# lalitkrajendran/photon

Hardware: AMD Instinct MI355X
Metric: Mrays/sec, 1e7-ray 256^3 BOS render (higher is better)
Workload: dtype f32

## Files before the change

### photon_amd/csrc/device_volume_coop.hpp

```cpp
#pragma once
#include "../../include/photon_philox.h"
#include "device_volume.hpp"

namespace photon {

enum PathSlot : int {
    PS_C_COHERENT,
    PS_C_HIT_CELL,
    PS_C_CELL_IN_TILE,
    PS_C_FETCH_UP,
    PS_C_FETCH_DOWN,
    PS_C_TILE_CLAMPED,
    PS_C_INCOHERENT,
    PS_C_INCOHERENT_LANES,
    PS_C_BRICK_PASS,
    PS_C_BRICK_FETCH,
    PS_C_BRICK_REUSED,
    PS_C_BRICK_CLAMPED,
    PS_C_BRICK_LANES,
    PS_C_GATHER_LANES,
    PS_C_SPIN_OUTSIDE,
    PS_C_SPIN_LOW,
    PS_C_SPIN_CAP,
    PS_L_COHERENT,
    PS_L_HIT_A,
    PS_L_HIT_B,
    PS_L_TILE_B_LANES,
    PS_L_FETCH,
    PS_L_FETCH_TWO,
    PS_L_FETCH_TO_B,
    PS_L_FETCH_DOWN,
    PS_L_BASE_AHEAD,
    PS_L_BASE_BEHIND,
    PS_L_TILE_CLAMPED,
    PS_L_NO_FREE_TILE,
    PS_L_OUT_OF_REACH,
    PS_L_MARK_INCOHERENT,
    PS_L_TILES_SKIPPED,
    PS_L_RETRY,
    PS_L_COHERENT_AGAIN,
    PS_L_INCOHERENT,
    PS_L_INCOHERENT_LANES,
    PS_L_BRICK_PASS,
    PS_L_BRICK_FETCH,
    PS_L_BRICK_REUSED,
    PS_L_BRICK_CLAMPED,
    PS_L_BRICK_LANES,
    PS_L_GATHER_LANES,
    PS_L_SPIN_OUTSIDE,
    PS_L_SPIN_CAP,
    PS_L_LOW,
    PS_L_REPAIR_LANES,
    PS_L_KEEP_PREV_LANES,
    PS_COUNT
};
constexpr int kPathSlots = PS_COUNT;
#ifndef PHOTON_PATH_STATS
#define PHOTON_PATH_STATS 0
#endif
#if PHOTON_PATH_STATS
__device__ unsigned long long g_path_stats[kPathSlots];
__device__ __forceinline__ void path_stat(PathSlot k, unsigned long long n = 1) {
    if ((int)(threadIdx.x & 63) == __ffsll((long long)ballot(true)) - 1) atomicAdd(&g_path_stats[k], n);
}
__device__ __forceinline__ void path_stat_if(PathSlot k, bool c) { if (c) path_stat(k); }
__device__ __forceinline__ void path_lanes(PathSlot k, unsigned long long mask) { if (mask != 0) path_stat(k, (unsigned long long)__popcll(mask)); }
#else
#define path_stat(...) ((void)0)
#define path_stat_if(...) ((void)0)
#define path_lanes(...) ((void)0)
#endif

#ifndef PHOTON_BRICK_PASSES
#define PHOTON_BRICK_PASSES 6
#endif
#ifndef PHOTON_LINEAR_TILE_LAYERS
#define PHOTON_LINEAR_TILE_LAYERS 16
#endif
#ifndef PHOTON_LINEAR_TILES
#define PHOTON_LINEAR_TILES 2
#endif
#ifndef PHOTON_TILE_RETRY_MASK
#define PHOTON_TILE_RETRY_MASK 15
#endif
#ifndef PHOTON_BRICK_PITCH
#define PHOTON_BRICK_PITCH 12
// ... 192 lines not shown
    }
#if PHOTON_PRIO_TAPS_DPP != PHOTON_PRIO_TAPS_LDS
    __builtin_amdgcn_s_setprio(PHOTON_PRIO_TAPS_LDS);
#endif
    f4 t[4] = {f4{t0.x, t0.y, t0.z, t0.w}, f4{t1.x, t1.y, t1.z, t1.w}, f4{t2.x, t2.y, t2.z, t2.w}, f4{t3.x, t3.y, t3.z, t3.w}};
    float w0 = wxy[0][0];
#pragma unroll
    for (int r = R; r < 16; r++) {
        const int b = r & 3, c = r >> 2;
#pragma unroll
        for (int a = 0; a < 4; a++) {
            const f4 ta = t[a];
            const float w = (a == 0 && b == 0) ? w0 : wxy[b][a];
            if (a == 0 && b == 0) s = f4{w * ta.x, w * ta.y, w * ta.z, w * ta.w};
            else s = f4{fmaf(w, ta.x, s.x), fmaf(w, ta.y, s.y), fmaf(w, ta.z, s.z), fmaf(w, ta.w, s.w)};
            asm volatile("" : "+v"(s.x), "+v"(s.y), "+v"(s.z), "+v"(s.w) : : "memory");
            if (r < 15) t[a] = ldtexel(blk + ((r + 1) >> 2) * 16 + ((r + 1) & 3) * 4 + a);
            asm volatile("" : "+v"(w0) : : "memory");
        }
        if (b == 3) {
            if (c == 0) acc = f4{wz[0] * s.x, wz[0] * s.y, wz[0] * s.z, wz[0] * s.w};
            else acc = f4{fmaf(wz[c], s.x, acc.x), fmaf(wz[c], s.y, acc.y), fmaf(wz[c], s.z, acc.z), fmaf(wz[c], s.w, acc.w)};
            asm volatile("" : "+v"(acc.x), "+v"(acc.y), "+v"(acc.z), "+v"(acc.w) : : "memory");
        }
    }
#if PHOTON_PRIO_TAPS_LDS != PHOTON_PRIO_BASE
    __builtin_amdgcn_s_setprio(PHOTON_PRIO_BASE);
#endif
    return acc;
}

__device__ __forceinline__ bool lane_of(unsigned long long mask) { return __builtin_amdgcn_inverse_ballot_w64(mask); }

struct Parked { int ti, tj, tk; int bi, bj, bk; f4 reg; int ci, cj, k0, coff; int ui, uj, uk; f4 more[3]; };
__device__ __forceinline__ Parked parked_none() {
    return Parked{0x7fffffff, 0x7fffffff, 0x7fffffff, 0x7fffffff, 0x7fffffff, 0x7fffffff, f4{0, 0, 0, 0}, 0x7fffffff, 0x7fffffff, 0, 0, 0x7fffffff, 0x7fffffff, 0x7fffffff, {f4{0, 0, 0, 0}, f4{0, 0, 0, 0}, f4{0, 0, 0, 0}}};
}

struct Lead { int i, j, k; };
__device__ __forceinline__ Lead lead_of(unsigned long long todo, float fi, float fj, float fk) {
    const int leader = __ffsll((long long)todo) - 1;
    return Lead{__builtin_amdgcn_readlane(__float_as_int(fi), leader), __builtin_amdgcn_readlane(__float_as_int(fj), leader),
                __builtin_amdgcn_readlane(__float_as_int(fk), leader)};
}
__device__ __forceinline__ unsigned long long same_block(const Lead &c, float fi, float fj, float fk) {
    return ballot(__float_as_int(fi) == c.i) & ballot(__float_as_int(fj) == c.j) & ballot(__float_as_int(fk) == c.k);
}

__device__ __forceinline__ f4 tex3d_cubic_coop(const VolumeDev &v, const f4 *__restrict__ tex, f4 *blk, unsigned long long need,
                                               float x, float y, float z, Parked &parked) {
    f4 *const brick = blk + tile_texels<2>();
    const float xg = x - 0.5f, yg = y - 0.5f, zg = z - 0.5f;
    const float fi = floorf(xg), fj = floorf(yg), fk = floorf(zg);
    float wx[4], wy[4], wz[4];
    bspline_weights(xg - fi, wx[0], wx[1], wx[2], wx[3]);
    bspline_weights(yg - fj, wy[0], wy[1], wy[2], wy[3]);
    bspline_weights(zg - fk, wz[0], wz[1], wz[2], wz[3]);
    const int lane = threadIdx.x & 63;
    if (need == 0) return f4{0, 0, 0, 0};
    {
        constexpr int TL = kCubicTileLayers;
        bool hit = false;
        if (parked.ti != 0x7fffffff) {
            asm volatile("");
            hit = ((ballot(__float_as_int(fi) == parked.ti) & ballot(__float_as_int(fj) == parked.tj) & ballot(__float_as_int(fk) == parked.tk)) & need) == need;
            path_stat_if(PS_C_HIT_CELL, hit);
        }
        if (!hit) {
            const Lead c = lead_of(need, fi, fj, fk);
            if ((same_block(c, fi, fj, fk) & need) == need) {
                const int ck = (int)__int_as_float(c.k);
                int dz = ck - parked.k0;
                if (c.i != parked.ci || c.j != parked.cj || (unsigned)dz > (unsigned)(TL - 4)) {
                    const int ci = (int)__int_as_float(c.i), cj = (int)__int_as_float(c.j);
                    const bool down = c.i == parked.ci && c.j == parked.cj && dz < 0;
                    const int k0 = down ? ck - (TL - 4) : ck;
                    path_stat(down ? PS_C_FETCH_DOWN : PS_C_FETCH_UP);
                    path_stat_if(PS_C_TILE_CLAMPED, ci < 1 || ci + 2 > v.nx - 1 || cj < 1 || cj + 2 > v.ny - 1 || k0 < 1 || k0 + TL - 2 > v.nz - 1);
                    __builtin_amdgcn_wave_barrier();
                    int l = lane;
                    asm volatile("" : "+v"(l));
                    const int tx = clampi(ci - 1 + (l & 3), 0, v.nx - 1), ty = clampi(cj - 1 + ((l >> 2) & 3), 0, v.ny - 1);
#pragma unroll
                    for (int j = 0; j < (TL + 3) / 4; j++) {
                        if (TL % 4 == 0 || j < TL / 4 || l < 16 * (TL % 4)) {
                            const int tz = clampi(k0 - 1 + (l >> 4) + 4 * j, 0, v.nz - 1);
                            const f4 t = ldtexel(tex + (unsigned)((tz * v.ny + ty) * v.nx + tx));
                            *reinterpret_cast<float4 *>(blk + l + 64 * j) = make_float4(t.x, t.y, t.z, t.w);
                        }
                    }
                    __builtin_amdgcn_wave_barrier();
                    parked.ci = c.i; parked.cj = c.j; parked.k0 = k0;
                    dz = ck - k0;
                } else {
                    path_stat(PS_C_CELL_IN_TILE);
                }
                parked.coff = dz * 16;
                parked.reg = ldtexel(blk + parked.coff + (lane & 15));
#pragma unroll
                for (int z = 1; z < kDppSlabs; z++) parked.more[z - 1] = ldtexel(blk + parked.coff + 16 * z + (lane & 15));
                parked.ti = c.i; parked.tj = c.j; parked.tk = c.k;
                hit = true;
            }
        }
        if (hit) {
            path_stat(PS_C_COHERENT);
            const f4 *cell = blk + parked.coff;
            const f4 acc = cubic_taps_hybrid(cell, parked.reg, parked.more, wx, wy, wz);
            __builtin_amdgcn_wave_barrier();
            return acc;
        }
        parked.ti = 0x7fffffff;
    }
    const int bi = (int)fi, bj = (int)fj, bk = (int)fk;
    f4 acc = f4{0, 0, 0, 0};
    bool done = !lane_of(need);
    unsigned long long todo = need;
    path_stat(PS_C_INCOHERENT);
    path_lanes(PS_C_INCOHERENT_LANES, need);
#pragma unroll 1
    for (int pass = 0; pass < PHOTON_BRICK_PASSES && todo != 0; pass++) {
        const int leader = __ffsll((long long)todo) - 1;
        const int ci = __builtin_amdgcn_readlane(bi, leader), cj = __builtin_amdgcn_readlane(bj, leader),
                  ck = __builtin_amdgcn_readlane(bk, leader);
        const int di = bi - ci + 2, dj = bj - cj + 2;
        const bool in_brick = !done && bk == ck && (unsigned)di <= 4u && (unsigned)dj <= 4u;
        path_stat(PS_C_BRICK_PASS);
        path_lanes(PS_C_BRICK_LANES, ballot(in_brick));
        path_stat(ci != parked.bi || cj != parked.bj || ck != parked.bk ? PS_C_BRICK_FETCH : PS_C_BRICK_REUSED);
        if (ci != parked.bi || cj != parked.bj || ck != parked.bk) {
            path_stat_if(PS_C_BRICK_CLAMPED, ci < 3 || ci + 4 > v.nx - 1 || cj < 3 || cj + 4 > v.ny - 1 || ck < 1 || ck + 2 > v.nz - 1);
            __builtin_amdgcn_wave_barrier();
            int l = lane;
            asm volatile("" : "+v"(l));
            const int slot = (l & 7) + ((l >> 3) & 7) * kBrickPitch;
#pragma unroll
            for (int j = 0; j < 4; j++) {
                const int t = l + 64 * j;
                const int tx = clampi(ci - 3 + (t & 7), 0, v.nx - 1), ty = clampi(cj - 3 + ((t >> 3) & 7), 0, v.ny - 1),
                          tz = clampi(ck - 1 + (t >> 6), 0, v.nz - 1);
// ... 27 lines not shown
    const float fi = floorf(xb), fj = floorf(yb), fk = floorf(zb);
    const float a = quant_weight(xb - fi, weight_scale, weight_inv), b = quant_weight(yb - fj, weight_scale, weight_inv),
                c = quant_weight(zb - fk, weight_scale, weight_inv);
    const int i = (int)fi, j = (int)fj, k = (int)fk;
    const int i0 = clampi(i, 0, nx - 1), i1 = clampi(i + 1, 0, nx - 1);
    const int j0 = clampi(j, 0, ny - 1), j1 = clampi(j + 1, 0, ny - 1);
    const int k0 = clampi(k, 0, nz - 1), k1 = clampi(k + 1, 0, nz - 1);
    auto row = [&](int kk, int jj) {
        const f4 *r = tex + (unsigned)((kk * ny + jj) * nx);
        f4 v = lerp4(ldtexel(r + i0), ldtexel(r + i1), a);
        asm volatile("" : "+v"(v.x), "+v"(v.y), "+v"(v.z), "+v"(v.w));
        return v;
    };
    const f4 c00 = row(k0, j0), c10 = row(k0, j1);
    f4 c0 = lerp4(c00, c10, b);
    asm volatile("" : "+v"(c0.x), "+v"(c0.y), "+v"(c0.z), "+v"(c0.w));
    const f4 c01 = row(k1, j0), c11 = row(k1, j1);
    const f4 c1 = lerp4(c01, c11, b);
    return lerp4(c0, c1, c);
}

__device__ __forceinline__ float uniformf(float x) {
    float s;
    asm("s_nop 0\n\tv_readfirstlane_b32 %0, %1\n\ts_nop 4" : "=s"(s) : "v"(x));
    return s;
}

__device__ __forceinline__ float pair_swap(float v) {
    return __int_as_float(__builtin_amdgcn_update_dpp(0, __float_as_int(v), 0xB1 , 0xF, 0xF, false));
}

template <bool QUANT, bool PIN = false>
__device__ __forceinline__ f4 tex3d_linear_coop(const VolumeDev &v, const f4 *__restrict__ tex, f4 *blk, unsigned long long need,
                                                float x, float y, float z, Parked &parked, unsigned tick = 0) {
    f4 *const brick = blk + tile_texels<1>();
    const float xb = x - 0.5f, yb = y - 0.5f, zb = z - 0.5f;
    const float fi = floorf(xb), fj = floorf(yb), fk = floorf(zb);
    float a = xb - fi, b = yb - fj, c = zb - fk;
    if (QUANT) {
        a = floorf(fmaf(a, v.weight_scale, 0.5f)) * v.weight_inv;

        b = floorf(fmaf(b, v.weight_scale, 0.5f)) * v.weight_inv;
        c = floorf(fmaf(c, v.weight_scale, 0.5f)) * v.weight_inv;
    }
    const int lane = threadIdx.x & 63;
    if (need == 0) return f4{0, 0, 0, 0};
    {
        constexpr int TL = PHOTON_LINEAR_TILE_LAYERS;
        constexpr int NT = PHOTON_LINEAR_TILES;
        static_assert(TL == 4 || TL == 8 || TL == 16, "PHOTON_LINEAR_TILE_LAYERS");
        static_assert(NT == 1 || NT == 2, "PHOTON_LINEAR_TILES");
        constexpr unsigned kDzMax = (unsigned)(TL - 2);
        constexpr int kIncoherent = 0x7ffffffe;
        const int fib = __float_as_int(fi), fjb = __float_as_int(fj);
        unsigned dzq = 0;
        unsigned long long ok_a = 0, ok_b = 0;
        bool hit = false;
        if (parked.ti != 0x7fffffff) {
            asm volatile("");
            dzq = (unsigned)(int)(fk - __int_as_float(parked.tk));
            ok_a = ballot(fib == parked.ti) & ballot(fjb == parked.tj) & ballot(dzq <= kDzMax);
            hit = (ok_a & need) == need;
            path_stat_if(PS_L_HIT_A, hit);
            if (NT == 2 && !hit && parked.ui < kIncoherent) {
                const unsigned dzu = (unsigned)(int)(fk - __int_as_float(parked.uk));
                ok_b = ballot(fib == parked.ui) & ballot(fjb == parked.uj) & ballot(dzu <= kDzMax);
                if (((ok_a | ok_b) & need) == need) {
                    hit = true;
                    path_stat(PS_L_HIT_B);
                    dzq = lane_of(ok_a) ? dzq : dzu + TL;
                }
            }
        }
        path_stat_if(PS_L_TILES_SKIPPED, !hit && parked.ui == kIncoherent && (tick & (unsigned)PHOTON_TILE_RETRY_MASK) != 0);
        path_stat_if(PS_L_RETRY, !hit && parked.ui == kIncoherent && (tick & (unsigned)PHOTON_TILE_RETRY_MASK) == 0);
        if (!hit && (parked.ui != kIncoherent || (tick & (unsigned)PHOTON_TILE_RETRY_MASK) == 0)) {
            const unsigned long long rest = need & ~(ok_a | ok_b);
            const Lead l1 = lead_of(rest, fi, fj, fk);
            const unsigned long long col1 = rest & ballot(fib == l1.i) & ballot(fjb == l1.j), rest2 = rest & ~col1;
            Lead l2 = l1;
            unsigned long long col2 = 0;
            int n_new = 1;
            if (rest2 != 0) {
                l2 = lead_of(rest2, fi, fj, fk);
                col2 = rest2 & ballot(fib == l2.i) & ballot(fjb == l2.j);
                n_new = (rest2 & ~col2) != 0 ? 3 : 2;
            }
            const bool free_a = (ok_a & need) == 0, free_b = NT == 2 && (ok_b & need) == 0;
            path_stat_if(PS_L_NO_FREE_TILE, n_new > (free_a ? 1 : 0) + (free_b ? 1 : 0));
            if (n_new <= (free_a ? 1 : 0) + (free_b ? 1 : 0)) {
                path_stat_if(PS_L_FETCH_TWO, n_new == 2);
#pragma unroll 1
                for (int j = 0; j < n_new; j++) {
                    path_stat(PS_L_FETCH);
                    const bool to_a = j == 0 && free_a;
                    const Lead ld = j == 0 ? l1 : l2;
                    const unsigned long long lanes = j == 0 ? col1 : col2;
                    const int oi = to_a ? parked.ti : parked.ui, oj = to_a ? parked.tj : parked.uj, ok = to_a ? parked.tk : parked.uk;
                    const float klf = __int_as_float(ld.k);
                    const bool behind = (lanes & ballot(fk < klf)) != 0, ahead = (lanes & ballot(fk > klf)) != 0;
                    const bool down = ld.i == oi && ld.j == oj && klf < __int_as_float(ok);
                    const int ci = (int)__int_as_float(ld.i), cj = (int)__int_as_float(ld.j);
                    const int base = (int)klf - (down ? (ahead ? TL - 3 : TL - 2) : (behind ? 1 : 0));
                    f4 *const tile = blk + (to_a ? 0 : 4 * TL);
                    path_stat_if(PS_L_FETCH_TO_B, !to_a);
                    path_stat_if(PS_L_FETCH_DOWN, down);
                    path_stat_if(PS_L_BASE_AHEAD, down && ahead);
                    path_stat_if(PS_L_BASE_BEHIND, !down && behind);
                    path_stat_if(PS_L_TILE_CLAMPED, ci < 0 || ci + 1 > v.nx - 1 || cj < 0 || cj + 1 > v.ny - 1 || base < 0 || base + TL - 1 > v.nz - 1);
                    __builtin_amdgcn_wave_barrier();
                    if (lane < 4 * TL) {
                        int l = lane;
                        if (PIN) asm volatile("" : "+v"(l));
                        const int tx = clampi(ci + (l & 1), 0, v.nx - 1), ty = clampi(cj + ((l >> 1) & 1), 0, v.ny - 1),
                                  tz = clampi(base + (l >> 2), 0, v.nz - 1);
                        const f4 t = ldtexel(tex + (unsigned)((tz * v.ny + ty) * v.nx + tx));
                        const f4 o = f4{pair_swap(t.x), pair_swap(t.y), pair_swap(t.z), pair_swap(t.w)};
                        const bool hi = (l & 1) != 0;
                        *reinterpret_cast<float4 *>(tile + l) = make_float4(hi ? t.x - o.x : t.x, hi ? t.y - o.y : t.y,
                                                                            hi ? t.z - o.z : t.z, hi ? t.w - o.w : t.w);
                    }
                    __builtin_amdgcn_wave_barrier();
                    const int basef = __float_as_int(uniformf((float)base));
                    if (to_a) { parked.ti = ld.i; parked.tj = ld.j; parked.tk = basef; }
                    else { parked.ui = ld.i; parked.uj = ld.j; parked.uk = basef; }
                }
                dzq = (unsigned)(int)(fk - __int_as_float(parked.tk));
                ok_a = ballot(fib == parked.ti) & ballot(fjb == parked.tj) & ballot(dzq <= kDzMax);
                if (NT == 2 && parked.ui < kIncoherent) {
                    const unsigned dzu = (unsigned)(int)(fk - __int_as_float(parked.uk));
                    ok_b = ballot(fib == parked.ui) & ballot(fjb == parked.uj) & ballot(dzu <= kDzMax);
                    dzq = lane_of(ok_a) ? dzq : dzu + TL;
                }
                hit = ((ok_a | ok_b) & need) == need;
                path_stat_if(PS_L_OUT_OF_REACH, !hit);
                path_stat_if(PS_L_COHERENT_AGAIN, hit && parked.ui == kIncoherent);
                if (hit && parked.ui == kIncoherent) parked.ui = 0x7fffffff;
            }
        }
        if (hit) {
            path_stat(PS_L_COHERENT);
            path_lanes(PS_L_TILE_B_LANES, need & ~ok_a);
            const f4 *q = blk + ((dzq & (unsigned)(NT * TL - 1)) << 2);
#if PHOTON_PRIO_BLEND != PHOTON_PRIO_BASE
            __builtin_amdgcn_s_setprio(PHOTON_PRIO_BLEND);
#endif
            const f4 c00 = lerp4d(ldtexel(q), ldtexel(q + 1), a), c10 = lerp4d(ldtexel(q + 2), ldtexel(q + 3), a);
            const f4 c01 = lerp4d(ldtexel(q + 4), ldtexel(q + 5), a), c11 = lerp4d(ldtexel(q + 6), ldtexel(q + 7), a);
            const f4 c0 = lerp4(c00, c10, b), c1 = lerp4(c01, c11, b);
            const f4 acc = lerp4(c0, c1, c);
#if PHOTON_PRIO_BLEND != PHOTON_PRIO_BASE
            __builtin_amdgcn_s_setprio(PHOTON_PRIO_BASE);
#endif
            __builtin_amdgcn_wave_barrier();
            return acc;
        }
        path_stat_if(PS_L_MARK_INCOHERENT, parked.ui != kIncoherent);
        parked.ti = 0x7fffffff;
        parked.ui = kIncoherent;
    }
    const int bi = (int)fi, bj = (int)fj, bk = (int)fk;
    f4 acc = f4{0, 0, 0, 0};
    bool done = !lane_of(need);
// ... 24 lines not shown
                const f4 tv = ldtexel(tex + (unsigned)((tz * v.ny + ty) * v.nx + tx));
                *reinterpret_cast<float4 *>(brick + slot + j * kBrickSlab) = make_float4(tv.x, tv.y, tv.z, tv.w);
            }
            __builtin_amdgcn_wave_barrier();
            parked.bi = ci; parked.bj = cj; parked.bk = ck;
        }
        if (in_brick) {
#if PHOTON_PRIO_BLEND != PHOTON_PRIO_BASE
            __builtin_amdgcn_s_setprio(PHOTON_PRIO_BLEND);
#endif
            const f4 *q = brick + (dj * kBrickPitch + di);
            const f4 c00 = lerp4(ldtexel(q), ldtexel(q + 1), a), c10 = lerp4(ldtexel(q + kBrickPitch), ldtexel(q + kBrickPitch + 1), a);
            const f4 c01 = lerp4(ldtexel(q + kBrickSlab), ldtexel(q + kBrickSlab + 1), a),
                     c11 = lerp4(ldtexel(q + kBrickSlab + kBrickPitch), ldtexel(q + kBrickSlab + kBrickPitch + 1), a);
            const f4 c0 = lerp4(c00, c10, b), c1 = lerp4(c01, c11, b);
            acc = lerp4(c0, c1, c);
#if PHOTON_PRIO_BLEND != PHOTON_PRIO_BASE
            __builtin_amdgcn_s_setprio(PHOTON_PRIO_BASE);
#endif
            done = true;
        }
        __builtin_amdgcn_wave_barrier();
        todo = ballot(!done);
    }
    path_lanes(PS_L_GATHER_LANES, ballot(!done));
    if (!done) acc = linear_gather_fn(tex, v.nx, v.ny, v.nz, x, y, z, v.weight_scale, v.weight_inv);
    return acc;
}

struct MarchU {
    float minx, miny, minz, maxx, maxy, maxz;
    float sx, sy, sz;
    float nxm2, nym2, nzm2;
    float fnx, fny, fnz;
    float step, data_min, spin_step;
    int nx, ny, nz;
};
__device__ __forceinline__ MarchU make_march_consts(const VolumeDev &v, f3 scale) {
    MarchU u;
    u.minx = uniformf(v.min_bound.x); u.miny = uniformf(v.min_bound.y); u.minz = uniformf(v.min_bound.z);
    u.maxx = uniformf(v.max_bound.x); u.maxy = uniformf(v.max_bound.y); u.maxz = uniformf(v.max_bound.z);
    u.sx = uniformf(scale.x); u.sy = uniformf(scale.y); u.sz = uniformf(scale.z);
    u.nxm2 = uniformf((float)(v.nx - 2)); u.nym2 = uniformf((float)(v.ny - 2)); u.nzm2 = uniformf((float)(v.nz - 2));
    u.fnx = uniformf((float)v.nx); u.fny = uniformf((float)v.ny); u.fnz = uniformf((float)v.nz);
    u.step = uniformf(v.step_size); u.data_min = uniformf(v.data_min);
    u.spin_step = uniformf(v.step_size / (1 + v.data_min));
    u.nx = v.nx; u.ny = v.ny; u.nz = v.nz;
    return u;
}
__device__ __forceinline__ f3 lookup_index_u(f3 pos, const MarchU &u) {
    const f3 off = mk3(pos.x - u.minx, pos.y - u.miny, pos.z - u.minz);
    const f3 fn = mk3(u.sx * off.x, u.sy * off.y, u.sz * off.z);
    return mk3(1 + fn.x * u.nxm2, 1 + fn.y * u.nym2, 1 + fn.z * u.nzm2);
}
__device__ __forceinline__ unsigned long long access_mask(const MarchU &u, f3 l) {
    return ~(ballot(l.x < 0) | ballot(l.y < 0) | ballot(l.z < 0) | ballot(l.x >= u.fnx) | ballot(l.y >= u.fny) | ballot(l.z >= u.fnz));
}
__device__ __forceinline__ unsigned long long inside_mask(f3 p, const MarchU &u) {
    return ~(ballot(p.x < u.minx) | ballot(p.y < u.miny) | ballot(p.z < u.minz) | ballot(p.x >= u.maxx) | ballot(p.y >= u.maxy) | ballot(p.z >= u.maxz));
}

struct WaveCount { unsigned iterations; unsigned samples; };
__device__ __forceinline__ void count_samples(MarchCount &mc, unsigned long long m) { if (lane_of(m)) mc.samples++; }
__device__ __forceinline__ void count_iterations(MarchCount &mc, unsigned long long m) { if (lane_of(m)) mc.iterations++; }
__device__ __forceinline__ void count_samples(WaveCount &mc, unsigned long long m) { mc.samples += (unsigned)__popcll(m); }
__device__ __forceinline__ void count_iterations(WaveCount &mc, unsigned long long m) { mc.iterations += (unsigned)__popcll(m); }

struct PrevVal {
    f4 v;
    __device__ __forceinline__ void init(f4 *, f4 x) { v = x; }
    __device__ __forceinline__ void set(f4 x) { v = x; }
    __device__ __forceinline__ f4 get() const { return v; }
};

template <int INTERP, bool QUANT, class CNT, bool PIN = false>
__device__ __forceinline__ f4 sample_coop(const VolumeDev &v, const f4 *__restrict__ tex, f4 *blk, unsigned long long need, f3 lookup,
                                          const PrevVal &prev, float data_min, CNT &mc, Parked &parked, unsigned tick = 0) {
    f4 val = INTERP == 1 ? tex3d_linear_coop<QUANT, PIN>(v, tex, blk, need, lookup.x, lookup.y, lookup.z, parked, tick)
                         : tex3d_cubic_coop(v, tex, blk, need, lookup.x, lookup.y, lookup.z, parked);
    count_samples(mc, need);
    if (INTERP == 1) {
        const unsigned long long low = need & ballot(val.w < data_min);
        if (low != 0) {
            const float ambient = 1.000277;
            const f4 val_prev = prev.get();
            const unsigned long long repair = low & ballot(val_prev.w == 0);
            path_stat(PS_L_LOW);
            path_lanes(PS_L_REPAIR_LANES, repair);
            path_lanes(PS_L_KEEP_PREV_LANES, low & ~repair);
            if (repair != 0) {
                count_samples(mc, repair);
                if (lane_of(repair)) {
                    const f4 t = linear_gather_fn(tex, v.nx, v.ny, v.nz, lookup.x, lookup.y, lookup.z - 1, v.weight_scale, v.weight_inv);
                    val = f4{t.x, t.y, t.z, ambient - 1};
                }
            }
            if (lane_of(low & ~repair)) val = val_prev;
        }
    }
    return val;
}

struct MarchResume {
    int loop_ctr, spins;
    f4 val_prev;
    unsigned max_trips;
    unsigned trips_base;
    bool fresh;
};
__device__ __forceinline__ MarchResume resume_fresh() { return MarchResume{0, 0, f4{0, 0, 0, 0}, ~0u, 0u, true}; }

template <int INTERP, bool SAVE, bool QUANT, class CNT>
__device__ __forceinline__ unsigned long long rk4_coop(bool active_lane, f3 &rpos, f3 &rdir, const VolumeDev &v,
                                                       const f4 *__restrict__ tex, f4 *blk, f3 scale, CNT &mc,
                                                       const InterDump &idump, MarchResume &rs) {
    const MarchU u = make_march_consts(v, scale);
    int loop_ctr = rs.loop_ctr;
    constexpr bool kSpinLds = PHOTON_SPINS_IN_LDS && INTERP == 1;
    int spins = rs.spins;
    int *const spin_slot = reinterpret_cast<int *>(blk + tile_texels<1>() + 2 * kBrickSlab) + (threadIdx.x & 63);
    if (kSpinLds) *spin_slot = spins;
    int *const ctr_slot = spin_slot + 64;
    if (kSpinLds) *ctr_slot = loop_ctr;
    unsigned trips = rs.trips_base;
    const unsigned trips_end = rs.max_trips == ~0u ? ~0u : trips + rs.max_trips;
    Parked parked = parked_none();
    PrevVal prev{};
    if (INTERP == 1) prev.init(blk, rs.val_prev);
    unsigned long long active = ballot(active_lane);
    unsigned long long first = active & ballot(loop_ctr == 0);
    while (active != 0 && trips < trips_end) {
        f3 lookup = lookup_index_u(rpos, u);
        const unsigned long long in_a = inside_mask(rpos, u);
        unsigned long long not_over = ~0ull;
        if (trips > (unsigned)kLoopMax) not_over = ~ballot((kSpinLds ? *ctr_slot : loop_ctr) > kLoopMax);
        trips++;
        if (SAVE && INTERP == 1) { if (lane_of(active & not_over)) record_intermediate(idump, kSpinLds ? *ctr_slot : loop_ctr, rpos, rdir); }
        const unsigned long long alive = active & not_over & (in_a | first);
        unsigned long long go = alive, spin = 0;
        if ((alive & ~in_a) != 0) {
            const unsigned long long access = access_mask(u, lookup);
            go = alive & access;
            spin = alive & ~access;
            path_lanes(INTERP == 1 ? PS_L_SPIN_OUTSIDE : PS_C_SPIN_OUTSIDE, spin);
        }
        f4 val = sample_coop<INTERP, QUANT, CNT, true>(v, tex, blk, go, lookup, prev, u.data_min, mc, parked, trips);
        if (INTERP == 2) {
            const unsigned long long low = go & ballot(val.w < u.data_min);
            path_lanes(PS_C_SPIN_LOW, low);
            spin |= low;
            go &= ~low;
        }
        active = alive;
        first &= ~go;
        if (spin != 0) {
            if (lane_of(spin)) {
                rpos = rpos + u.spin_step * rdir;
                if (kSpinLds) { spins = *spin_slot + 1; *spin_slot = spins; } else spins++;
            }
            path_lanes(INTERP == 1 ? PS_L_SPIN_CAP : PS_C_SPIN_CAP, spin & ballot(spins > kSpinMax));
            active &= ~(spin & ballot(spins > kSpinMax));
        }
        if (kSpinLds) { if (lane_of(go)) atomicAdd(ctr_slot, 1); } else loop_ctr += lane_of(go) ? 1 : 0;
        const float n_a = val.w + 1;
        const float delta_t = div_nr(u.step, n_a);
        f3 T_n = n_a * rdir;
        const f3 A = delta_t * mk3(n_a * val.x, n_a * val.y, n_a * val.z);
        f3 spos = rpos + (0.5f * delta_t) * T_n + (0.125f * delta_t) * A;
        if (INTERP == 1) prev.set(f4{val.x, val.y, val.z, n_a - 1});
        lookup = lookup_index_u(spos, u);
        unsigned long long in = inside_mask(spos, u);
        active &= ~go | in;
        go &= in;
        val = sample_coop<INTERP, QUANT, CNT, true>(v, tex, blk, go, lookup, prev, u.data_min, mc, parked, trips);
        const float n_b = val.w + 1;
        const f3 B = delta_t * mk3(n_b * val.x, n_b * val.y, n_b * val.z);
        spos = rpos + delta_t * T_n + (0.5f * delta_t) * B;
        if (INTERP == 1) prev.set(f4{val.x, val.y, val.z, n_b - 1});
        lookup = lookup_index_u(spos, u);
        in = inside_mask(spos, u);
        active &= ~go | in;
        go &= in;
        val = sample_coop<INTERP, QUANT, CNT, true>(v, tex, blk, go, lookup, prev, u.data_min, mc, parked, trips);
        const float n_c = val.w + 1;
        const f3 C = delta_t * mk3(n_c * val.x, n_c * val.y, n_c * val.z);
        if (INTERP == 1) prev.set(f4{val.x, val.y, val.z, n_c - 1});
        if (lane_of(go)) {
            rpos = rpos + delta_t * (T_n + (float)(1 / 6.0) * (A + 2.0f * B));
            T_n = T_n + (float)(1 / 6.0) * (A + 4.0f * B + C);
            rdir = normalize_nr(div_nr(T_n, INTERP == 1 ? n_a : n_c));
        }
        count_iterations(mc, go);
        if (INTERP == 1 && spin != 0) { if (lane_of(spin)) prev.set(f4{0, 0, 0, 0}); }
    }
    rs.loop_ctr = kSpinLds ? *ctr_slot : loop_ctr; rs.spins = kSpinLds ? *spin_slot : spins;
    if (INTERP == 1) rs.val_prev = prev.get();
    return active;
}

struct GradNoise { int on; float std; unsigned long long seed, ray_id; };

template <int INTERP, bool SAVE, bool NOISE, bool QUANT, class CNT>
__device__ __forceinline__ unsigned long long euler_coop(bool active_lane, f3 &rpos, f3 &rdir, const VolumeDev &v,
                                                         const f4 *__restrict__ tex, f4 *blk, f3 scale, CNT &mc,
                                                         const GradNoise &gn, const InterDump &idump, MarchResume &rs) {
    const MarchU u = make_march_consts(v, scale);
    int loop_ctr = rs.loop_ctr, spins = rs.spins;
    unsigned trips = rs.trips_base;
    const unsigned trips_end = rs.max_trips == ~0u ? ~0u : trips + rs.max_trips;
    Parked parked = parked_none();
    PrevVal prev{};
    if (INTERP == 1) prev.init(blk, rs.val_prev);
    unsigned long long active = ballot(active_lane);
    unsigned long long first = active & ballot(loop_ctr == 0);
    while (active != 0 && trips < trips_end) {
        const f3 lookup = lookup_index_u(rpos, u);
        const unsigned long long in_a = inside_mask(rpos, u);
        unsigned long long not_over = ~0ull;
        if (trips > (unsigned)kLoopMax) not_over = ~ballot(loop_ctr > kLoopMax);
        trips++;
        if (SAVE && INTERP == 1) { if (lane_of(active & not_over)) record_intermediate(idump, loop_ctr, rpos, rdir); }
        const unsigned long long alive = active & not_over & (in_a | first);
        unsigned long long go = alive, spin = 0;
        if (INTERP == 1 && (alive & ~in_a) != 0) {
            const unsigned long long access = access_mask(u, lookup);
            go = alive & access;
            spin = alive & ~access;
            path_lanes(PS_L_SPIN_OUTSIDE, spin);
        }
        f4 val = sample_coop<INTERP, QUANT, CNT>(v, tex, blk, go, lookup, prev, u.data_min, mc, parked, trips);
        if (INTERP == 2) {
            const unsigned long long low = go & ballot(val.w < u.data_min);
            path_lanes(PS_C_SPIN_LOW, low);
            spin |= low;
            go &= ~low;
        }
        active = alive;
        first &= ~go;
        if (spin != 0) {
            if (lane_of(spin)) {
                rpos = rpos + u.spin_step * rdir;
                spins++;
            }
            path_lanes(INTERP == 1 ? PS_L_SPIN_CAP : PS_C_SPIN_CAP, spin & ballot(spins > kSpinMax));
            active &= ~(spin & ballot(spins > kSpinMax));
        }
        if (INTERP == 1) {
            if (NOISE) {
                float n0, n1;
                photon_normal2(gn.seed, gn.ray_id, (unsigned)loop_ctr, PHOTON_STREAM_NGRAD_NOISE, &n0, &n1);
                val.x += n0 * gn.std;
                val.y += n1 * gn.std;
            }
            if (lane_of(go)) {
                const float current_n = 1 + val.w;
                rdir = rdir + u.step * mk3(val.x, val.y, val.z);
                rpos = rpos + div_nr(u.step, current_n) * rdir;
                prev.set(val);
            }
        } else {
            if (lane_of(go)) {
                rdir = normalize_nr(rdir + u.step * mk3(val.x, val.y, val.z));
                const float n = 1 + val.w;
                rpos = rpos + div_nr(rdir * u.step, n);
            }
        }
        loop_ctr += lane_of(go) ? 1 : 0;
        count_iterations(mc, go);
    }
    rs.loop_ctr = loop_ctr; rs.spins = spins;
    if (INTERP == 1) rs.val_prev = prev.get();
    return active;
}

template <int ALGO, int INTERP, bool SAVE, bool NOISE, bool QUANT, class CNT>
__device__ __forceinline__ unsigned long long trace_volume_coop(bool has_ray, f3 &pos_io, f3 &dir_io, const VolumeDev &v,
                                                                const f4 *__restrict__ tex, f4 *blk, CNT &mc,
                                                                const GradNoise &gn, const InterDump &idump, MarchResume &rs) {
    const f3 mn = v.min_bound, mx = v.max_bound;
    const f3 scale = mk3(1.0f / (mx.x - mn.x), 1.0f / (mx.y - mn.y), 1.0f / (mx.z - mn.z));
    bool active = has_ray;
    if (has_ray && rs.fresh) {
        f3 pos = pos_io;
        const f3 dir = dir_io;
        if (pos.x <= mn.x || pos.y <= mn.y || pos.z <= mn.z || pos.x >= mx.x || pos.y >= mx.y || pos.z >= mx.z) {
            if (!intersect_with_volume(pos, dir, mn, mx)) active = false;
        }
        if (active) pos_io = pos;
    }
#if PHOTON_PRIO_BASE > 0
    __builtin_amdgcn_s_setprio(PHOTON_PRIO_BASE);
#endif
    unsigned long long still;
    if (ALGO == 1) still = euler_coop<INTERP, SAVE, NOISE, QUANT, CNT>(active, pos_io, dir_io, v, tex, blk, scale, mc, gn, idump, rs);
    else still = rk4_coop<INTERP, SAVE, QUANT, CNT>(active, pos_io, dir_io, v, tex, blk, scale, mc, idump, rs);
#if PHOTON_PRIO_BASE > 0
    __builtin_amdgcn_s_setprio(0);
#endif
    return still;
}

}
```

### photon_amd/path_stats.py

```python
from __future__ import annotations

import ctypes
import os
import re

HEADER = os.path.join(os.path.dirname(os.path.abspath(__file__)), "csrc", "device_volume_coop.hpp")

SLOTS = (
    "C_COHERENT", "C_HIT_CELL", "C_CELL_IN_TILE", "C_FETCH_UP", "C_FETCH_DOWN", "C_TILE_CLAMPED",
    "C_INCOHERENT", "C_INCOHERENT_LANES", "C_BRICK_PASS", "C_BRICK_FETCH", "C_BRICK_REUSED", "C_BRICK_CLAMPED",
    "C_BRICK_LANES", "C_GATHER_LANES", "C_SPIN_OUTSIDE", "C_SPIN_LOW", "C_SPIN_CAP",
    "L_COHERENT", "L_HIT_A", "L_HIT_B", "L_TILE_B_LANES", "L_FETCH", "L_FETCH_TWO", "L_FETCH_TO_B", "L_FETCH_DOWN",
    "L_BASE_AHEAD", "L_BASE_BEHIND", "L_TILE_CLAMPED", "L_NO_FREE_TILE", "L_OUT_OF_REACH", "L_MARK_INCOHERENT",
    "L_TILES_SKIPPED", "L_RETRY", "L_COHERENT_AGAIN", "L_INCOHERENT", "L_INCOHERENT_LANES", "L_BRICK_PASS",
    "L_BRICK_FETCH", "L_BRICK_REUSED", "L_BRICK_CLAMPED", "L_BRICK_LANES", "L_GATHER_LANES", "L_SPIN_OUTSIDE",
    "L_SPIN_CAP", "L_LOW", "L_REPAIR_LANES", "L_KEEP_PREV_LANES",
)

PATH_STATS_FLAGS = ("-DPHOTON_PATH_STATS=1",)


def header_slots(path: str = HEADER):
    with open(path) as f:
        text = f.read()
    body = re.search(r"enum PathSlot\s*:\s*int\s*\{(.*?)\};", text, re.S).group(1)
    names = re.findall(r"^\s*PS_(\w+)\s*,", body, re.M)
    assert names and names[-1] != "COUNT"
    return tuple(names)


def read(lib) -> dict:
    f = lib.lib.photon_debug_path_stats
    f.argtypes = [ctypes.c_void_p, ctypes.c_int]
    f.restype = ctypes.c_int
    out = (ctypes.c_ulonglong * len(SLOTS))()
    rc = f(ctypes.cast(out, ctypes.c_void_p), len(SLOTS))
    if rc != 0:
        raise RuntimeError(f"photon_debug_path_stats failed ({rc})")
    return dict(zip(SLOTS, (int(v) for v in out)))
```

Before: 191.9.

## Skip volume bounds test when lanes sample an unclamped parked tile

Tile lookup (locate) is hoisted ahead of the inside-volume test. When every candidate lane hits a parked tile or cell that was fetched without clamping, the per-lane bounding-box ballots are skipped, and a flag bit stored in the parked tile base or offset marks that state. The access mask now derives its float bounds from scalar ints rather than stored floats. The tile-hit ballots are reused inside the sampler, so the bookkeeping is not done twice. The cost is extra ballots at fetch time to decide whether a tile was clamped, plus the added complexity of the bit-tagging.

```diff
diff --git a/photon_amd/csrc/device_volume_coop.hpp b/photon_amd/csrc/device_volume_coop.hpp
--- a/photon_amd/csrc/device_volume_coop.hpp
+++ b/photon_amd/csrc/device_volume_coop.hpp
@@ -22,6 +22,7 @@
     PS_C_SPIN_OUTSIDE,
     PS_C_SPIN_LOW,
     PS_C_SPIN_CAP,
+    PS_C_BOX_FROM_CELL,
     PS_L_COHERENT,
     PS_L_HIT_A,
     PS_L_HIT_B,
@@ -52,6 +53,7 @@
     PS_L_LOW,
     PS_L_REPAIR_LANES,
     PS_L_KEEP_PREV_LANES,
+    PS_L_BOX_FROM_TILE,
     PS_COUNT
 };
 constexpr int kPathSlots = PS_COUNT;
@@ -310,6 +312,8 @@
 
 __device__ __forceinline__ bool lane_of(unsigned long long mask) { return __builtin_amdgcn_inverse_ballot_w64(mask); }
 
+constexpr int kBoxCoff = (int)0x80000000, kCoffMask = 0x0fffffff, kBoxBase = 1;
+__device__ __forceinline__ float tile_base(int tk) { return __int_as_float(tk & ~kBoxBase); }
 struct Parked { int ti, tj, tk; int bi, bj, bk; f4 reg; int ci, cj, k0, coff; int ui, uj, uk; f4 more[3]; };
 __device__ __forceinline__ Parked parked_none() {
     return Parked{0x7fffffff, 0x7fffffff, 0x7fffffff, 0x7fffffff, 0x7fffffff, 0x7fffffff, f4{0, 0, 0, 0}, 0x7fffffff, 0x7fffffff, 0, 0, 0x7fffffff, 0x7fffffff, 0x7fffffff, {f4{0, 0, 0, 0}, f4{0, 0, 0, 0}, f4{0, 0, 0, 0}}};
@@ -325,11 +329,49 @@
     return ballot(__float_as_int(fi) == c.i) & ballot(__float_as_int(fj) == c.j) & ballot(__float_as_int(fk) == c.k);
 }
 
+#ifndef PHOTON_BOX_FROM_CELL
+#define PHOTON_BOX_FROM_CELL 1
+#endif
+struct Located { float xg, yg, zg, fi, fj, fk; unsigned dzq; int how; unsigned long long ok_a; };
+constexpr int kServedA = 1, kServedAB = 3;
+constexpr int kIncoherent = 0x7ffffffe;
+template <int INTERP>
+__device__ __forceinline__ Located locate(f3 lookup, const Parked &parked, unsigned long long cand) {
+    Located at;
+    at.xg = lookup.x - 0.5f; at.yg = lookup.y - 0.5f; at.zg = lookup.z - 0.5f;
+    at.fi = floorf(at.xg); at.fj = floorf(at.yg); at.fk = floorf(at.zg);
+    at.dzq = 0;
+    at.how = 0;
+    at.ok_a = 0;
+    if (parked.ti != 0x7fffffff) {
+        asm volatile("");
+        const int fib = __float_as_int(at.fi), fjb = __float_as_int(at.fj);
+        if (INTERP == 2) {
+            at.how = ((ballot(fib == parked.ti) & ballot(fjb == parked.tj) & ballot(__float_as_int(at.fk) == parked.tk)) & cand) == cand ? kServedA : 0;
+        } else {
+            constexpr int TL = PHOTON_LINEAR_TILE_LAYERS;
+            constexpr unsigned kDzMax = (unsigned)(TL - 2);
+            at.dzq = (unsigned)(int)(at.fk - tile_base(parked.tk));
+            at.ok_a = ballot(fib == parked.ti) & ballot(fjb == parked.tj) & ballot(at.dzq <= kDzMax);
+            at.how = (at.ok_a & cand) == cand ? kServedA : 0;
+            if (PHOTON_LINEAR_TILES == 2 && at.how == 0 && parked.ui < kIncoherent) {
+                const unsigned dzu = (unsigned)(int)(at.fk - tile_base(parked.uk));
+                const unsigned long long ok_b = ballot(fib == parked.ui) & ballot(fjb == parked.uj) & ballot(dzu <= kDzMax);
+                if (((at.ok_a | ok_b) & cand) == cand) {
+                    at.how = kServedAB;
+                    at.dzq = lane_of(at.ok_a) ? at.dzq : dzu + TL;
+                }
+            }
+        }
+    }
+    return at;
+}
+
 __device__ __forceinline__ f4 tex3d_cubic_coop(const VolumeDev &v, const f4 *__restrict__ tex, f4 *blk, unsigned long long need,
-                                               float x, float y, float z, Parked &parked) {
+                                               float x, float y, float z, const Located &at, Parked &parked) {
     f4 *const brick = blk + tile_texels<2>();
-    const float xg = x - 0.5f, yg = y - 0.5f, zg = z - 0.5f;
-    const float fi = floorf(xg), fj = floorf(yg), fk = floorf(zg);
+    const float xg = at.xg, yg = at.yg, zg = at.zg;
+    const float fi = at.fi, fj = at.fj, fk = at.fk;
     float wx[4], wy[4], wz[4];
     bspline_weights(xg - fi, wx[0], wx[1], wx[2], wx[3]);
     bspline_weights(yg - fj, wy[0], wy[1], wy[2], wy[3]);
@@ -339,11 +381,8 @@
     {
         constexpr int TL = kCubicTileLayers;
         bool hit = false;
-        if (parked.ti != 0x7fffffff) {
-            asm volatile("");
-            hit = ((ballot(__float_as_int(fi) == parked.ti) & ballot(__float_as_int(fj) == parked.tj) & ballot(__float_as_int(fk) == parked.tk)) & need) == need;
-            path_stat_if(PS_C_HIT_CELL, hit);
-        }
+        hit = at.how != 0;
+        path_stat_if(PS_C_HIT_CELL, hit);
         if (!hit) {
             const Lead c = lead_of(need, fi, fj, fk);
             if ((same_block(c, fi, fj, fk) & need) == need) {
@@ -358,7 +397,9 @@
                     __builtin_amdgcn_wave_barrier();
                     int l = lane;
                     asm volatile("" : "+v"(l));
-                    const int tx = clampi(ci - 1 + (l & 3), 0, v.nx - 1), ty = clampi(cj - 1 + ((l >> 2) & 3), 0, v.ny - 1);
+                    const int ux = ci - 1 + (l & 3), uy = cj - 1 + ((l >> 2) & 3);
+                    const int tx = clampi(ux, 0, v.nx - 1), ty = clampi(uy, 0, v.ny - 1);
+                    const bool clamped = PHOTON_BOX_FROM_CELL && ((ballot(tx != ux) | ballot(ty != uy)) != 0 || k0 < 1 || k0 + TL - 2 > v.nz - 1);
 #pragma unroll
                     for (int j = 0; j < (TL + 3) / 4; j++) {
                         if (TL % 4 == 0 || j < TL / 4 || l < 16 * (TL % 4)) {
@@ -370,20 +411,21 @@
                     __builtin_amdgcn_wave_barrier();
                     parked.ci = c.i; parked.cj = c.j; parked.k0 = k0;
                     dz = ck - k0;
+                    parked.coff = PHOTON_BOX_FROM_CELL && !clamped ? kBoxCoff : 0;
                 } else {
                     path_stat(PS_C_CELL_IN_TILE);
                 }
-                parked.coff = dz * 16;
-                parked.reg = ldtexel(blk + parked.coff + (lane & 15));
-#pragma unroll
-                for (int z = 1; z < kDppSlabs; z++) parked.more[z - 1] = ldtexel(blk + parked.coff + 16 * z + (lane & 15));
+                parked.coff = dz * 16 | (parked.coff & kBoxCoff);
+                parked.reg = ldtexel(blk + dz * 16 + (lane & 15));
+#pragma unroll
+                for (int z = 1; z < kDppSlabs; z++) parked.more[z - 1] = ldtexel(blk + dz * 16 + 16 * z + (lane & 15));
                 parked.ti = c.i; parked.tj = c.j; parked.tk = c.k;
                 hit = true;
             }
         }
         if (hit) {
             path_stat(PS_C_COHERENT);
-            const f4 *cell = blk + parked.coff;
+            const f4 *cell = blk + (parked.coff & kCoffMask);
             const f4 acc = cubic_taps_hybrid(cell, parked.reg, parked.more, wx, wy, wz);
             __builtin_amdgcn_wave_barrier();
             return acc;
@@ -477,10 +519,10 @@
 
 template <bool QUANT, bool PIN = false>
 __device__ __forceinline__ f4 tex3d_linear_coop(const VolumeDev &v, const f4 *__restrict__ tex, f4 *blk, unsigned long long need,
-                                                float x, float y, float z, Parked &parked, unsigned tick = 0) {
+                                                float x, float y, float z, const Located &at, Parked &parked, unsigned tick = 0) {
     f4 *const brick = blk + tile_texels<1>();
-    const float xb = x - 0.5f, yb = y - 0.5f, zb = z - 0.5f;
-    const float fi = floorf(xb), fj = floorf(yb), fk = floorf(zb);
+    const float xb = at.xg, yb = at.yg, zb = at.zg;
+    const float fi = at.fi, fj = at.fj, fk = at.fk;
     float a = xb - fi, b = yb - fj, c = zb - fk;
     if (QUANT) {
         a = floorf(fmaf(a, v.weight_scale, 0.5f)) * v.weight_inv;
@@ -496,19 +538,19 @@
         static_assert(TL == 4 || TL == 8 || TL == 16, "PHOTON_LINEAR_TILE_LAYERS");
         static_assert(NT == 1 || NT == 2, "PHOTON_LINEAR_TILES");
         constexpr unsigned kDzMax = (unsigned)(TL - 2);
-        constexpr int kIncoherent = 0x7ffffffe;
         const int fib = __float_as_int(fi), fjb = __float_as_int(fj);
-        unsigned dzq = 0;
-        unsigned long long ok_a = 0, ok_b = 0;
-        bool hit = false;
-        if (parked.ti != 0x7fffffff) {
+        unsigned dzq = at.dzq;
+        unsigned long long ok_a = at.ok_a, ok_b = 0;
+        bool hit = at.how != 0;
+        path_stat_if(at.how == kServedAB ? PS_L_HIT_B : PS_L_HIT_A, hit);
+        if (!hit && parked.ti != 0x7fffffff) {
             asm volatile("");
-            dzq = (unsigned)(int)(fk - __int_as_float(parked.tk));
+            dzq = (unsigned)(int)(fk - tile_base(parked.tk));
             ok_a = ballot(fib == parked.ti) & ballot(fjb == parked.tj) & ballot(dzq <= kDzMax);
             hit = (ok_a & need) == need;
             path_stat_if(PS_L_HIT_A, hit);
             if (NT == 2 && !hit && parked.ui < kIncoherent) {
-                const unsigned dzu = (unsigned)(int)(fk - __int_as_float(parked.uk));
+                const unsigned dzu = (unsigned)(int)(fk - tile_base(parked.uk));
                 ok_b = ballot(fib == parked.ui) & ballot(fjb == parked.uj) & ballot(dzu <= kDzMax);
                 if (((ok_a | ok_b) & need) == need) {
                     hit = true;
@@ -544,7 +586,7 @@
                     const int oi = to_a ? parked.ti : parked.ui, oj = to_a ? parked.tj : parked.uj, ok = to_a ? parked.tk : parked.uk;
                     const float klf = __int_as_float(ld.k);
                     const bool behind = (lanes & ballot(fk < klf)) != 0, ahead = (lanes & ballot(fk > klf)) != 0;
-                    const bool down = ld.i == oi && ld.j == oj && klf < __int_as_float(ok);
+                    const bool down = ld.i == oi && ld.j == oj && klf < tile_base(ok);
                     const int ci = (int)__int_as_float(ld.i), cj = (int)__int_as_float(ld.j);
                     const int base = (int)klf - (down ? (ahead ? TL - 3 : TL - 2) : (behind ? 1 : 0));
                     f4 *const tile = blk + (to_a ? 0 : 4 * TL);
@@ -553,10 +595,17 @@
                     path_stat_if(PS_L_BASE_AHEAD, down && ahead);
                     path_stat_if(PS_L_BASE_BEHIND, !down && behind);
                     path_stat_if(PS_L_TILE_CLAMPED, ci < 0 || ci + 1 > v.nx - 1 || cj < 0 || cj + 1 > v.ny - 1 || base < 0 || base + TL - 1 > v.nz - 1);
+                    bool outer = false;
+                    int lp = lane;
+                    if (PHOTON_BOX_FROM_CELL) {
+                        asm volatile("" : "+v"(lp));
+                        outer = base < 1 || base + TL > v.nz - 1 ||
+                                (ballot((unsigned)(ci - 1 + 3 * (lp & 1)) >= (unsigned)v.nx) | ballot((unsigned)(cj - 1 + 3 * ((lp >> 1) & 1)) >= (unsigned)v.ny)) != 0;
+                    }
                     __builtin_amdgcn_wave_barrier();
                     if (lane < 4 * TL) {
-                        int l = lane;
-                        if (PIN) asm volatile("" : "+v"(l));
+                        int l = PHOTON_BOX_FROM_CELL ? lp : lane;
+                        if (PIN && !PHOTON_BOX_FROM_CELL) asm volatile("" : "+v"(l));
                         const int tx = clampi(ci + (l & 1), 0, v.nx - 1), ty = clampi(cj + ((l >> 1) & 1), 0, v.ny - 1),
                                   tz = clampi(base + (l >> 2), 0, v.nz - 1);
                         const f4 t = ldtexel(tex + (unsigned)((tz * v.ny + ty) * v.nx + tx));
@@ -566,14 +615,14 @@
                                                                             hi ? t.z - o.z : t.z, hi ? t.w - o.w : t.w);
                     }
                     __builtin_amdgcn_wave_barrier();
-                    const int basef = __float_as_int(uniformf((float)base));
+                    const int basef = __float_as_int(uniformf((float)base)) | (PHOTON_BOX_FROM_CELL && !outer ? kBoxBase : 0);
                     if (to_a) { parked.ti = ld.i; parked.tj = ld.j; parked.tk = basef; }
                     else { parked.ui = ld.i; parked.uj = ld.j; parked.uk = basef; }
                 }
-                dzq = (unsigned)(int)(fk - __int_as_float(parked.tk));
+                dzq = (unsigned)(int)(fk - tile_base(parked.tk));
                 ok_a = ballot(fib == parked.ti) & ballot(fjb == parked.tj) & ballot(dzq <= kDzMax);
                 if (NT == 2 && parked.ui < kIncoherent) {
-                    const unsigned dzu = (unsigned)(int)(fk - __int_as_float(parked.uk));
+                    const unsigned dzu = (unsigned)(int)(fk - tile_base(parked.uk));
                     ok_b = ballot(fib == parked.ui) & ballot(fjb == parked.uj) & ballot(dzu <= kDzMax);
                     dzq = lane_of(ok_a) ? dzq : dzu + TL;
                 }
@@ -664,7 +713,6 @@
     float minx, miny, minz, maxx, maxy, maxz;
     float sx, sy, sz;
     float nxm2, nym2, nzm2;
-    float fnx, fny, fnz;
     float step, data_min, spin_step;
     int nx, ny, nz;
 };
@@ -674,7 +722,6 @@
     u.maxx = uniformf(v.max_bound.x); u.maxy = uniformf(v.max_bound.y); u.maxz = uniformf(v.max_bound.z);
     u.sx = uniformf(scale.x); u.sy = uniformf(scale.y); u.sz = uniformf(scale.z);
     u.nxm2 = uniformf((float)(v.nx - 2)); u.nym2 = uniformf((float)(v.ny - 2)); u.nzm2 = uniformf((float)(v.nz - 2));
-    u.fnx = uniformf((float)v.nx); u.fny = uniformf((float)v.ny); u.fnz = uniformf((float)v.nz);
     u.step = uniformf(v.step_size); u.data_min = uniformf(v.data_min);
     u.spin_step = uniformf(v.step_size / (1 + v.data_min));
     u.nx = v.nx; u.ny = v.ny; u.nz = v.nz;
@@ -686,10 +733,29 @@
     return mk3(1 + fn.x * u.nxm2, 1 + fn.y * u.nym2, 1 + fn.z * u.nzm2);
 }
 __device__ __forceinline__ unsigned long long access_mask(const MarchU &u, f3 l) {
-    return ~(ballot(l.x < 0) | ballot(l.y < 0) | ballot(l.z < 0) | ballot(l.x >= u.fnx) | ballot(l.y >= u.fny) | ballot(l.z >= u.fnz));
+    int nx = u.nx, ny = u.ny, nz = u.nz;
+    asm volatile("" : "+s"(nx), "+s"(ny), "+s"(nz));
+    return ~(ballot(l.x < 0) | ballot(l.y < 0) | ballot(l.z < 0) | ballot(l.x >= (float)nx) | ballot(l.y >= (float)ny) | ballot(l.z >= (float)nz));
 }
 __device__ __forceinline__ unsigned long long inside_mask(f3 p, const MarchU &u) {
     return ~(ballot(p.x < u.minx) | ballot(p.y < u.miny) | ballot(p.z < u.minz) | ballot(p.x >= u.maxx) | ballot(p.y >= u.maxy) | ballot(p.z >= u.maxz));
+}
+template <int INTERP>
+__device__ __forceinline__ unsigned long long inside_or_parked(const Located &at, const Parked &parked, unsigned long long cand, f3 p, const MarchU &u) {
+#if PHOTON_BOX_FROM_CELL
+    if (INTERP == 2) {
+        if (at.how != 0 && parked.coff < 0) {
+            path_stat_if(PS_C_BOX_FROM_CELL, cand != 0);
+            return cand;
+        }
+    } else {
+        if (((at.how == kServedAB ? parked.tk & parked.uk : parked.tk) & at.how & kBoxBase) != 0) {
+            path_stat_if(PS_L_BOX_FROM_TILE, cand != 0);
+            return cand;
+        }
+    }
+#endif
+    return inside_mask(p, u);
 }
 
 struct WaveCount { unsigned iterations; unsigned samples; };
@@ -706,10 +772,10 @@
 };
 
 template <int INTERP, bool QUANT, class CNT, bool PIN = false>
-__device__ __forceinline__ f4 sample_coop(const VolumeDev &v, const f4 *__restrict__ tex, f4 *blk, unsigned long long need, f3 lookup,
+__device__ __forceinline__ f4 sample_coop(const VolumeDev &v, const f4 *__restrict__ tex, f4 *blk, unsigned long long need, f3 lookup, const Located &at,
                                           const PrevVal &prev, float data_min, CNT &mc, Parked &parked, unsigned tick = 0) {
-    f4 val = INTERP == 1 ? tex3d_linear_coop<QUANT, PIN>(v, tex, blk, need, lookup.x, lookup.y, lookup.z, parked, tick)
-                         : tex3d_cubic_coop(v, tex, blk, need, lookup.x, lookup.y, lookup.z, parked);
+    f4 val = INTERP == 1 ? tex3d_linear_coop<QUANT, PIN>(v, tex, blk, need, lookup.x, lookup.y, lookup.z, at, parked, tick)
+                         : tex3d_cubic_coop(v, tex, blk, need, lookup.x, lookup.y, lookup.z, at, parked);
     count_samples(mc, need);
     if (INTERP == 1) {
         const unsigned long long low = need & ballot(val.w < data_min);
@@ -763,10 +829,11 @@
     unsigned long long first = active & ballot(loop_ctr == 0);
     while (active != 0 && trips < trips_end) {
         f3 lookup = lookup_index_u(rpos, u);
-        const unsigned long long in_a = inside_mask(rpos, u);
         unsigned long long not_over = ~0ull;
         if (trips > (unsigned)kLoopMax) not_over = ~ballot((kSpinLds ? *ctr_slot : loop_ctr) > kLoopMax);
         trips++;
+        Located at = locate<INTERP>(lookup, parked, active);
+        const unsigned long long in_a = inside_or_parked<INTERP>(at, parked, active, rpos, u);
         if (SAVE && INTERP == 1) { if (lane_of(active & not_over)) record_intermediate(idump, kSpinLds ? *ctr_slot : loop_ctr, rpos, rdir); }
         const unsigned long long alive = active & not_over & (in_a | first);
         unsigned long long go = alive, spin = 0;
@@ -776,7 +843,7 @@
             spin = alive & ~access;
             path_lanes(INTERP == 1 ? PS_L_SPIN_OUTSIDE : PS_C_SPIN_OUTSIDE, spin);
         }
-        f4 val = sample_coop<INTERP, QUANT, CNT, true>(v, tex, blk, go, lookup, prev, u.data_min, mc, parked, trips);
+        f4 val = sample_coop<INTERP, QUANT, CNT, true>(v, tex, blk, go, lookup, at, prev, u.data_min, mc, parked, trips);
         if (INTERP == 2) {
             const unsigned long long low = go & ballot(val.w < u.data_min);
             path_lanes(PS_C_SPIN_LOW, low);
@@ -801,19 +868,21 @@
         f3 spos = rpos + (0.5f * delta_t) * T_n + (0.125f * delta_t) * A;
         if (INTERP == 1) prev.set(f4{val.x, val.y, val.z, n_a - 1});
         lookup = lookup_index_u(spos, u);
-        unsigned long long in = inside_mask(spos, u);
+        at = locate<INTERP>(lookup, parked, go);
+        unsigned long long in = inside_or_parked<INTERP>(at, parked, go, spos, u);
         active &= ~go | in;
         go &= in;
-        val = sample_coop<INTERP, QUANT, CNT, true>(v, tex, blk, go, lookup, prev, u.data_min, mc, parked, trips);
+        val = sample_coop<INTERP, QUANT, CNT, true>(v, tex, blk, go, lookup, at, prev, u.data_min, mc, parked, trips);
         const float n_b = val.w + 1;
         const f3 B = delta_t * mk3(n_b * val.x, n_b * val.y, n_b * val.z);
         spos = rpos + delta_t * T_n + (0.5f * delta_t) * B;
         if (INTERP == 1) prev.set(f4{val.x, val.y, val.z, n_b - 1});
         lookup = lookup_index_u(spos, u);
-        in = inside_mask(spos, u);
+        at = locate<INTERP>(lookup, parked, go);
+        in = inside_or_parked<INTERP>(at, parked, go, spos, u);
         active &= ~go | in;
         go &= in;
-        val = sample_coop<INTERP, QUANT, CNT, true>(v, tex, blk, go, lookup, prev, u.data_min, mc, parked, trips);
+        val = sample_coop<INTERP, QUANT, CNT, true>(v, tex, blk, go, lookup, at, prev, u.data_min, mc, parked, trips);
         const float n_c = val.w + 1;
         const f3 C = delta_t * mk3(n_c * val.x, n_c * val.y, n_c * val.z);
         if (INTERP == 1) prev.set(f4{val.x, val.y, val.z, n_c - 1});
@@ -847,10 +916,11 @@
     unsigned long long first = active & ballot(loop_ctr == 0);
     while (active != 0 && trips < trips_end) {
         const f3 lookup = lookup_index_u(rpos, u);
-        const unsigned long long in_a = inside_mask(rpos, u);
         unsigned long long not_over = ~0ull;
         if (trips > (unsigned)kLoopMax) not_over = ~ballot(loop_ctr > kLoopMax);
         trips++;
+        const Located at = locate<INTERP>(lookup, parked, active);
+        const unsigned long long in_a = inside_or_parked<INTERP>(at, parked, active, rpos, u);
         if (SAVE && INTERP == 1) { if (lane_of(active & not_over)) record_intermediate(idump, loop_ctr, rpos, rdir); }
         const unsigned long long alive = active & not_over & (in_a | first);
         unsigned long long go = alive, spin = 0;
@@ -860,7 +930,7 @@
             spin = alive & ~access;
             path_lanes(PS_L_SPIN_OUTSIDE, spin);
         }
-        f4 val = sample_coop<INTERP, QUANT, CNT>(v, tex, blk, go, lookup, prev, u.data_min, mc, parked, trips);
+        f4 val = sample_coop<INTERP, QUANT, CNT>(v, tex, blk, go, lookup, at, prev, u.data_min, mc, parked, trips);
         if (INTERP == 2) {
             const unsigned long long low = go & ballot(val.w < u.data_min);
             path_lanes(PS_C_SPIN_LOW, low);
@@ -910,7 +980,7 @@
                                                                 const f4 *__restrict__ tex, f4 *blk, CNT &mc,
                                                                 const GradNoise &gn, const InterDump &idump, MarchResume &rs) {
     const f3 mn = v.min_bound, mx = v.max_bound;
-    const f3 scale = mk3(1.0f / (mx.x - mn.x), 1.0f / (mx.y - mn.y), 1.0f / (mx.z - mn.z));
+    const f3 scale = mk3(uniformf(1.0f / (mx.x - mn.x)), uniformf(1.0f / (mx.y - mn.y)), uniformf(1.0f / (mx.z - mn.z)));
     bool active = has_ray;
     if (has_ray && rs.fresh) {
         f3 pos = pos_io;
diff --git a/photon_amd/path_stats.py b/photon_amd/path_stats.py
--- a/photon_amd/path_stats.py
+++ b/photon_amd/path_stats.py
@@ -9,12 +9,12 @@
 SLOTS = (
     "C_COHERENT", "C_HIT_CELL", "C_CELL_IN_TILE", "C_FETCH_UP", "C_FETCH_DOWN", "C_TILE_CLAMPED",
     "C_INCOHERENT", "C_INCOHERENT_LANES", "C_BRICK_PASS", "C_BRICK_FETCH", "C_BRICK_REUSED", "C_BRICK_CLAMPED",
-    "C_BRICK_LANES", "C_GATHER_LANES", "C_SPIN_OUTSIDE", "C_SPIN_LOW", "C_SPIN_CAP",
+    "C_BRICK_LANES", "C_GATHER_LANES", "C_SPIN_OUTSIDE", "C_SPIN_LOW", "C_SPIN_CAP", "C_BOX_FROM_CELL",
     "L_COHERENT", "L_HIT_A", "L_HIT_B", "L_TILE_B_LANES", "L_FETCH", "L_FETCH_TWO", "L_FETCH_TO_B", "L_FETCH_DOWN",
     "L_BASE_AHEAD", "L_BASE_BEHIND", "L_TILE_CLAMPED", "L_NO_FREE_TILE", "L_OUT_OF_REACH", "L_MARK_INCOHERENT",
     "L_TILES_SKIPPED", "L_RETRY", "L_COHERENT_AGAIN", "L_INCOHERENT", "L_INCOHERENT_LANES", "L_BRICK_PASS",
     "L_BRICK_FETCH", "L_BRICK_REUSED", "L_BRICK_CLAMPED", "L_BRICK_LANES", "L_GATHER_LANES", "L_SPIN_OUTSIDE",
-    "L_SPIN_CAP", "L_LOW", "L_REPAIR_LANES", "L_KEEP_PREV_LANES",
+    "L_SPIN_CAP", "L_LOW", "L_REPAIR_LANES", "L_KEEP_PREV_LANES", "L_BOX_FROM_TILE",
 )
 
 PATH_STATS_FLAGS = ("-DPHOTON_PATH_STATS=1",)
```

Result: no change. 191.6 (-0.1%).
